# Rikorose/DeepFilterNet

Measured on AMD Instinct MI355X. Metric: 48 kHz audio frames/sec (hop=480), DeepFilterNet3 enhance(), higher is better.
Workload: dtype f32 (storage and accumulation; GRU projections / recurrences, the fused DF-encoder convolutions and the pointwise halves of the ERB separable convolutions as fp16-split MFMAs: x = hi + lo in f16, hi*hi + hi*lo + lo*hi on v_mfma_f32_16x16x32_f16, ~2^-21 relative; see exact_fp32_ms_per_step); 1 GPU; DeepFilterNet3 (recalled shipped shape, conv_ch=64) enhance(pad=True), batch=256 clips x 10 s @48 kHz per GPU, 1002 STFT frames per clip; batch_per_gpu=256, global_batch=256, parallelism=clips sharded over 1 GPU(s); no collective, inputs_resident_in_hbm=True

## Files before the change

deepfilternet_amd/csrc/dfx_nn_kernels.h:

```cpp
#pragma once

#include "dfx_common.h"

#include <type_traits>

#define DFX_ACT_NONE 0
#define DFX_ACT_RELU 1
#define DFX_ACT_TANH 2
#define DFX_ACT_SIGMOID 3

static __device__ __forceinline__ float dfx_sigmoid(float x) { return 1.f / (1.f + expf(-x)); }
static __device__ __forceinline__ float dfx_act(float v, int act) {
    if (act == DFX_ACT_RELU) return fmaxf(v, 0.f);
    if (act == DFX_ACT_TANH) return tanhf(v);
    if (act == DFX_ACT_SIGMOID) return dfx_sigmoid(v);
    return v;
}

template <int I, int N, typename F>
static __device__ __forceinline__ void dfx_static_for(F &&f) {
    if constexpr (I < N) {
        f(std::integral_constant<int, I>{});
        dfx_static_for<I + 1, N>(f);
    }
// ... 333 lines not shown
#pragma unroll
        for (int ks = 0; ks < CPL; ++ks) areg[nt][ks] = A.wt[(16 * (ks >> 2) + 4 * q + (ks & 3)) * C + 16 * nt + jl];
    float4 bias0[NT], biasr[NT];
#pragma unroll
    for (int nt = 0; nt < NT; ++nt) {
        bias0[nt] = reinterpret_cast<const float4 *>(A.bias0)[4 * nt + q];
        biasr[nt] = reinterpret_cast<const float4 *>(A.bias)[4 * nt + q];
    }
    __syncthreads();
    const int64_t Tn = A.t_end - A.t_begin;
    const int64_t total = A.B * Tn * A.Fout;
    const int64_t ntiles = (total + 15) / 16;
    for (int64_t tile = (int64_t)blockIdx.x * 4 + wave; tile < ntiles; tile += (int64_t)gridDim.x * 4) {
        const int64_t lpos = tile * 16 + jl;
        const bool valid = lpos < total;
        const int64_t rl = lpos / A.Fout;
        const int fo = (int)(lpos - rl * A.Fout);
        const int64_t b = rl / Tn, t = A.t_begin + (rl - b * Tn);
        const int64_t pos = (b * A.T + t) * A.Fout + fo;
        float u[CPL];
#pragma unroll
        for (int i = 0; i < CPL; ++i) u[i] = 0.f;
#pragma unroll
        for (int j = 0; j < 3; ++j) {
            const int fi = fo * A.stride + j - 1;
            const bool ok = valid && fi >= 0 && fi < A.Fin;
            float bv[5], c0v[CPL];
            dfx_c0_patch(A.feat, b, t, fi, ok, A.T, A.Fin, A.L, q, bv);
            dfx_c0_tile<C>(areg0, bias0, bv, ok, c0v);
#pragma unroll
            for (int nt = 0; nt < NT; ++nt) {
                const float4 w = dws[j * (C / 4) + 4 * nt + q];
                u[4 * nt + 0] += w.x * c0v[4 * nt + 0];
                u[4 * nt + 1] += w.y * c0v[4 * nt + 1];
                u[4 * nt + 2] += w.z * c0v[4 * nt + 2];
                u[4 * nt + 3] += w.w * c0v[4 * nt + 3];
            }
        }
        f32x4 acc[NT];
#pragma unroll
        for (int nt = 0; nt < NT; ++nt) acc[nt] = f32x4{0.f, 0.f, 0.f, 0.f};
#pragma unroll
        for (int ks = 0; ks < CPL; ++ks)
#pragma unroll
            for (int nt = 0; nt < NT; ++nt) acc[nt] = __builtin_amdgcn_mfma_f32_16x16x4f32(areg[nt][ks], u[ks], acc[nt], 0, 0, 0);
        if (valid) {
            float4 *op = reinterpret_cast<float4 *>(A.out + pos * C + 4 * q);
#pragma unroll
            for (int nt = 0; nt < NT; ++nt)
                op[4 * nt] = make_float4(fmaxf(acc[nt][0] + biasr[nt].x, 0.f), fmaxf(acc[nt][1] + biasr[nt].y, 0.f),
                                         fmaxf(acc[nt][2] + biasr[nt].z, 0.f), fmaxf(acc[nt][3] + biasr[nt].w, 0.f));
        }
    }
}

static __device__ __forceinline__ void dfx_c0_patch_load(const float *__restrict__ feat, int64_t b, int64_t t, int f, bool valid,
                                                         int64_t T, int Fin, int L, int q, float2 (&raw)[4], int64_t Ts = 0) {
    if (Ts <= 0) Ts = T;
#pragma unroll
    for (int i = 0; i < 4; ++i) {
        const int tap = 4 * q + i, kt = tap / 3, kf = tap - 3 * kt;
        const int64_t tau = t - 2 + kt, tin = tau + L;
        const int fin = f - 1 + kf;
        float2 v = make_float2(0.f, 0.f);
        if (valid && tap < 9 && tau >= 0 && tin < T && fin >= 0 && fin < Fin)
            v = *reinterpret_cast<const float2 *>(feat + ((b * Ts + tin) * Fin + fin) * 2);
        raw[i] = v;
    }
}

template <int C>
static __device__ __forceinline__ void dfx_c0_tile_h3(const dfx_h8 (&w0h)[C / 16], const dfx_h8 (&w0l)[C / 16],
                                                      const float4 (&bias0)[C / 16], float unscale0, const float2 (&raw)[4],
                                                      bool keep, float (&dst)[C / 4], float &amax) {
    constexpr int NT = C / 16;
    float x[8];
#pragma unroll
    for (int i = 0; i < 4; ++i) x[2 * i] = raw[i].x, x[2 * i + 1] = raw[i].y;
    dfx_h8 ph, pl;
    dfx_split8_g(x, ph, pl, amax);
    f32x4 acc[NT];
#pragma unroll
    for (int nt = 0; nt < NT; ++nt) acc[nt] = dfx_mfma_16x16x32_f16(w0l[nt], ph, f32x4{0.f, 0.f, 0.f, 0.f});
#pragma unroll
    for (int nt = 0; nt < NT; ++nt) acc[nt] = dfx_mfma_16x16x32_f16(w0h[nt], pl, acc[nt]);
#pragma unroll
    for (int nt = 0; nt < NT; ++nt) acc[nt] = dfx_mfma_16x16x32_f16(w0h[nt], ph, acc[nt]);
#pragma unroll
    for (int nt = 0; nt < NT; ++nt) {
        dst[4 * nt + 0] = keep ? fmaxf(acc[nt][0] * unscale0 + bias0[nt].x, 0.f) : 0.f;
        dst[4 * nt + 1] = keep ? fmaxf(acc[nt][1] * unscale0 + bias0[nt].y, 0.f) : 0.f;
        dst[4 * nt + 2] = keep ? fmaxf(acc[nt][2] * unscale0 + bias0[nt].z, 0.f) : 0.f;
        dst[4 * nt + 3] = keep ? fmaxf(acc[nt][3] * unscale0 + bias0[nt].w, 0.f) : 0.f;
    }
}

struct DfxC01hArgs {
    const float *feat;
    const dfx_h8 *w0f;
    const float *bias0;
    const float *dw;
    const dfx_h8 *wpf;
    const float *bias;
    float *out;
    int64_t B, T;
    int Fin, Fout, stride, L;
    float unscale0, unscale;
    int64_t t_begin;
    int64_t t_end;
    unsigned int *err;
    int64_t feat_T = 0;
};

template <int C>
#ifndef DFX_C01_MINB
#define DFX_C01_MINB 3
#endif
#ifndef DFX_C01_PIN
#define DFX_C01_PIN 0
#endif
#ifndef DFX_C01_EPI_BATCH
#define DFX_C01_EPI_BATCH 2
#endif
__global__ void __launch_bounds__(DFX_PW_THREADS, DFX_C01_MINB) dfx_k_df_conv01_h3(DfxC01hArgs A) {
    constexpr int CPL = C / 4, NT = C / 16, KC = C >= 32 ? C / 32 : 1, C4 = C / 4;
    static_assert(C % 32 == 0, "one k-chunk is 32 channels");
    __shared__ float4 dws[3 * C4];
    __shared__ float4 b0s[C4], b1s[C4];
    __shared__ dfx_h8 wps[NT * KC * 2 * 64];
    const int tid = threadIdx.x, lane = tid & 63, wave = tid >> 6, q = lane >> 4, jl = lane & 15;
    for (int i = tid; i < 3 * C4; i += DFX_PW_THREADS) dws[i] = reinterpret_cast<const float4 *>(A.dw)[i];
    for (int i = tid; i < C4; i += DFX_PW_THREADS) {
        b0s[i] = reinterpret_cast<const float4 *>(A.bias0)[i];
        b1s[i] = reinterpret_cast<const float4 *>(A.bias)[i];
    }
    for (int i = tid; i < NT * KC * 2 * 64; i += DFX_PW_THREADS) wps[i] = A.wpf[i];
    dfx_h8 w0h[NT], w0l[NT];
#pragma unroll
    for (int nt = 0; nt < NT; ++nt) {
        w0h[nt] = A.w0f[(nt * 2 + 0) * 64 + lane];
        w0l[nt] = A.w0f[(nt * 2 + 1) * 64 + lane];
    }
    __syncthreads();
    const unsigned Tn = (unsigned)(A.t_end - A.t_begin);
    const unsigned NF = (unsigned)A.B * Tn;
    const int TPF = (A.Fout + 15) >> 4;
    const unsigned nwaves = gridDim.x * 4;
    const int T32 = (int)A.T, Fin = A.Fin, Lk = A.L;
    int tdt[4], tdf[4];
    bool tok[4];
#pragma unroll
    for (int i = 0; i < 4; ++i) {
        const int tap = 4 * q + i, kt = tap / 3;
        tok[i] = tap < 9;
        tdt[i] = kt - 2 + Lk;
        tdf[i] = tap - 3 * kt - 1;
    }
    float2 raw[3][4];
    bool okj[3];
    const unsigned wid = (unsigned)blockIdx.x * 4 + (unsigned)dfx_wave_uniform(wave);
    const unsigned step_fr = nwaves / (unsigned)TPF;
    const int step_ft = (int)(nwaves - step_fr * (unsigned)TPF);
    unsigned nfr = wid / (unsigned)TPF;
    int nft = (int)(wid - nfr * (unsigned)TPF), nb = 0, nt_ = 0;
    bool nlive = nfr < NF;
    auto settle = [&]() {
        if (nlive) {
            nb = (int)(nfr / Tn);
            nt_ = (int)A.t_begin + (int)(nfr - (unsigned)nb * Tn);
        }
    };
    settle();
    auto issue = [&](int j) {
        const int fo = nft * 16 + jl;
        const int fi = fo * A.stride + j - 1;
        okj[j] = nlive && fo < A.Fout && fi >= 0 && fi < Fin;
        const float2 *clip = reinterpret_cast<const float2 *>(A.feat) + (int64_t)nb * (A.feat_T > 0 ? A.feat_T : (int64_t)T32) * Fin;
#pragma unroll
        for (int i = 0; i < 4; ++i) {
            const int tin = nt_ + tdt[i], fin = fi + tdf[i];
            float2 v = make_float2(0.f, 0.f);
            if (okj[j] && tok[i] && tin - Lk >= 0 && tin < T32 && fin >= 0 && fin < Fin) v = clip[tin * Fin + fin];
            raw[j][i] = v;
        }
    };
    float amax = 0.f;
#pragma unroll
    for (int j = 0; j < 3; ++j) issue(j);
    while (nlive) {
        const int fo_c = nft * 16 + jl;
        const bool valid = fo_c < A.Fout;
        const int64_t pos = ((int64_t)nb * T32 + nt_) * A.Fout + fo_c;
        nft += step_ft;
        nfr += step_fr;
        if (nft >= TPF) nft -= TPF, ++nfr;
        nlive = nfr < NF;
        settle();
        float u[CPL];
#pragma unroll
        for (int i = 0; i < CPL; ++i) u[i] = 0.f;
#pragma unroll
        for (int j = 0; j < 3; ++j) {
            float x[8];
#pragma unroll
            for (int i = 0; i < 4; ++i) x[2 * i] = raw[j][i].x, x[2 * i + 1] = raw[j][i].y;
            const bool keep = okj[j];
            dfx_h8 ph, pl;
            dfx_split8_g(x, ph, pl, amax);
            issue(j);
            f32x4 acc[NT];
#pragma unroll
            for (int nt = 0; nt < NT; ++nt) acc[nt] = dfx_mfma_16x16x32_f16(w0l[nt], ph, f32x4{0.f, 0.f, 0.f, 0.f});
#pragma unroll
            for (int nt = 0; nt < NT; ++nt) acc[nt] = dfx_mfma_16x16x32_f16(w0h[nt], pl, acc[nt]);
#pragma unroll
            for (int nt = 0; nt < NT; ++nt) acc[nt] = dfx_mfma_16x16x32_f16(w0h[nt], ph, acc[nt]);
#if DFX_C01_PIN
#pragma unroll
            for (int n0 = 0; n0 < NT; n0 += DFX_C01_EPI_BATCH) {
                float4 bz[DFX_C01_EPI_BATCH], w[DFX_C01_EPI_BATCH];
#pragma unroll
                for (int d = 0; d < DFX_C01_EPI_BATCH; ++d) {
                    bz[d] = b0s[4 * (n0 + d) + q], w[d] = dws[j * C4 + 4 * (n0 + d) + q];
                    DFX_OPAQUE(bz[d].x);
                    DFX_OPAQUE(bz[d].y);
                    DFX_OPAQUE(bz[d].z);
                    DFX_OPAQUE(bz[d].w);
                    DFX_OPAQUE(w[d].x);
                    DFX_OPAQUE(w[d].y);
                    DFX_OPAQUE(w[d].z);
                    DFX_OPAQUE(w[d].w);
                }
#pragma unroll
                for (int d = 0; d < DFX_C01_EPI_BATCH; ++d) {
                    const int nt = n0 + d;
                    u[4 * nt + 0] += w[d].x * (keep ? fmaxf(acc[nt][0] * A.unscale0 + bz[d].x, 0.f) : 0.f);
                    u[4 * nt + 1] += w[d].y * (keep ? fmaxf(acc[nt][1] * A.unscale0 + bz[d].y, 0.f) : 0.f);
                    u[4 * nt + 2] += w[d].z * (keep ? fmaxf(acc[nt][2] * A.unscale0 + bz[d].z, 0.f) : 0.f);
                    u[4 * nt + 3] += w[d].w * (keep ? fmaxf(acc[nt][3] * A.unscale0 + bz[d].w, 0.f) : 0.f);
                }
            }
#else
#pragma unroll
            for (int nt = 0; nt < NT; ++nt) {
                const float4 bz = b0s[4 * nt + q], w = dws[j * C4 + 4 * nt + q];
                u[4 * nt + 0] += w.x * (keep ? fmaxf(acc[nt][0] * A.unscale0 + bz.x, 0.f) : 0.f);
                u[4 * nt + 1] += w.y * (keep ? fmaxf(acc[nt][1] * A.unscale0 + bz.y, 0.f) : 0.f);
                u[4 * nt + 2] += w.z * (keep ? fmaxf(acc[nt][2] * A.unscale0 + bz.z, 0.f) : 0.f);
                u[4 * nt + 3] += w.w * (keep ? fmaxf(acc[nt][3] * A.unscale0 + bz.w, 0.f) : 0.f);
            }
#endif
        }
        dfx_h8 uh[KC], ul[KC];
#pragma unroll
        for (int kc = 0; kc < KC; ++kc) dfx_split8_g(u + 8 * kc, uh[kc], ul[kc], amax);
        float4 *op = reinterpret_cast<float4 *>(A.out + pos * C + 4 * q);
        int zoff = 0;
        DFX_OPAQUE(zoff);
        const dfx_h8 *wpl_ = wps + lane + zoff;
#pragma unroll
        for (int nt = 0; nt < NT; ++nt) {
            f32x4 aa = f32x4{0.f, 0.f, 0.f, 0.f}, ab = aa, ac = aa;
#pragma unroll
            for (int kc = 0; kc < KC; ++kc) {
                const dfx_h8 wh = wpl_[((nt * KC + kc) * 2 + 0) * 64], wl = wpl_[((nt * KC + kc) * 2 + 1) * 64];
                aa = dfx_mfma_16x16x32_f16(wl, uh[kc], aa);
                ab = dfx_mfma_16x16x32_f16(wh, ul[kc], ab);
                ac = dfx_mfma_16x16x32_f16(wh, uh[kc], ac);
            }
            if (valid) {
                const float4 bz = b1s[4 * nt + q];
                op[4 * nt] = make_float4(fmaxf(((aa[0] + ab[0]) + ac[0]) * A.unscale + bz.x, 0.f),
                                         fmaxf(((aa[1] + ab[1]) + ac[1]) * A.unscale + bz.y, 0.f),
                                         fmaxf(((aa[2] + ab[2]) + ac[2]) * A.unscale + bz.z, 0.f),
                                         fmaxf(((aa[3] + ab[3]) + ac[3]) * A.unscale + bz.w, 0.f));
            }
        }
    }
    if (amax >= DFX_H3_LIMIT && A.err) dfx_raise(A.err + 1);
}

struct DfxDfEncArgs {
    const float *feat;
    const dfx_h8 *w0f;
    const float *bias0;
    const float *dw;
    const dfx_h8 *wpf;
    const float *bias;
    const dfx_h8 *wfc;
    const dfx_h8 *win;
    const float *e3;
    float *emb_in;
    float *xa;
    int64_t B, T;
    int Fin, Fout, stride, L;
    int cpg;
    int nsplit = 1;
    float unscale0, unscale, unscale_fc, unscale_in;
    int64_t t_begin, t_end;
    unsigned int *err;
    int64_t feat_T = 0;
};

template <int C>
__global__ void __launch_bounds__(DFX_PW_THREADS, 3) dfx_k_df_enc_h3(DfxDfEncArgs A) {
    constexpr int CPL = C / 4, NT = C / 16, KC = C / 32, C4 = C / 4;
    static_assert(C % 32 == 0, "one k-chunk is 32 channels");
    __shared__ float4 dws[3 * C4];
    __shared__ float4 b0s[C4], b1s[C4];
    __shared__ dfx_h8 wps[NT * KC * 2 * 64];
    __shared__ dfx_h8 w0s[NT * 2 * 64];
    __shared__ __attribute__((aligned(16))) int tis[4 * DFX_PW_THREADS];
    __shared__ float4 uns[NT * DFX_PW_THREADS];
    const int tid = threadIdx.x, lane = tid & 63, wave = tid >> 6, q = lane >> 4, jl = lane & 15;
    for (int i = tid; i < 3 * C4; i += DFX_PW_THREADS) dws[i] = reinterpret_cast<const float4 *>(A.dw)[i];
    for (int i = tid; i < C4; i += DFX_PW_THREADS) {
        b0s[i] = reinterpret_cast<const float4 *>(A.bias0)[i];
        b1s[i] = reinterpret_cast<const float4 *>(A.bias)[i];
    }
    for (int i = tid; i < NT * KC * 2 * 64; i += DFX_PW_THREADS) wps[i] = A.wpf[i];
    for (int i = tid; i < NT * 2 * 64; i += DFX_PW_THREADS) w0s[i] = A.w0f[i];
    __syncthreads();
    const unsigned Tn = (unsigned)(A.t_end - A.t_begin), NFR = (unsigned)A.B * Tn, nsp = (unsigned)A.nsplit, ntiles = ((NFR + 15) >> 4) * nsp;
    const int bpp = A.Fout / A.nsplit;
    const unsigned nwaves = gridDim.x * 4;
    const int T32 = (int)A.T, Fin = A.Fin, Lk = A.L, Fout = A.Fout, emb = Fout * C / A.cpg / 2;
    const int64_t fT = A.feat_T > 0 ? A.feat_T : (int64_t)T32;
    {
        int ti[4];
#pragma unroll
        for (int i = 0; i < 4; ++i) {
            const int tap = 4 * q + i, kt = tap / 3;
            ti[i] = (kt - 2 + Lk + 64) | ((tap - 3 * kt) << 8) | ((tap < 9 ? 1 : 0) << 16);
        }
#pragma unroll
        for (int i = 0; i < 4; ++i) tis[4 * tid + i] = ti[i];
    }
    float amax = 0.f;
    for (unsigned tile = (unsigned)blockIdx.x * 4 + (unsigned)dfx_wave_uniform(wave); tile < ntiles; tile += nwaves) {
        const unsigned ftile = tile / nsp, part = tile - ftile * nsp;
        const int fo0 = (int)part * bpp, fo1 = fo0 + bpp;
        const unsigned rl = (ftile << 4) + (unsigned)jl, b = rl / Tn;
        const int t = (int)A.t_begin + (int)(rl - b * Tn);
        const bool live = rl < NFR;
        const float2 *feat2 = reinterpret_cast<const float2 *>(A.feat);
        const unsigned cbase = b * (unsigned)fT * (unsigned)Fin;
        const unsigned row = b * (unsigned)T32 + (unsigned)t;
        float2 raw[2][4];
        auto issue_to = [&](float2 (&dst)[4], int j, int fo) {
            const int fi = fo * A.stride + j - 1;
            const bool ok = live && fo < fo1 && fi >= 0 && fi < Fin;
            int zt = tid;
            DFX_OPAQUE(zt);
            const int tinfo[4] = {tis[4 * zt], tis[4 * zt + 1], tis[4 * zt + 2], tis[4 * zt + 3]};
#pragma unroll
            for (int i = 0; i < 4; ++i) {
                const int tin = t + (tinfo[i] & 0xff) - 64, fin = fi + ((tinfo[i] >> 8) & 0xff) - 1;
                float2 v = make_float2(0.f, 0.f);
                if (ok && (tinfo[i] >> 16) && tin - Lk >= 0 && tin < T32 && fin >= 0 && fin < Fin) v = feat2[cbase + (unsigned)(tin * Fin + fin)];
                dst[i] = v;
            }
        };
        auto c0_tile = [&](auto jc, auto addc, auto nextc, int fo, float2 (&rw)[4], float (&u)[CPL], bool refill) {
            constexpr int j = decltype(jc)::value;
            constexpr bool ADD = decltype(addc)::value, NEXT = decltype(nextc)::value;
            float x[8];
#pragma unroll
            for (int i = 0; i < 4; ++i) x[2 * i] = rw[i].x, x[2 * i + 1] = rw[i].y;
            const int fi = fo * A.stride + j - 1;
            const bool keep = live && fi >= 0 && fi < Fin;
            dfx_h8 ph, pl;
            dfx_split8_g(x, ph, pl, amax);
            if (refill) issue_to(rw, j, fo + 1);
            int z0 = 0;
            DFX_OPAQUE(z0);
            dfx_h8 w0h[NT], w0l[NT];
#pragma unroll
            for (int nt = 0; nt < NT; ++nt) {
                w0h[nt] = w0s[(nt * 2 + 0) * 64 + lane + z0];
                w0l[nt] = w0s[(nt * 2 + 1) * 64 + lane + z0];
            }
            f32x4 acc[NT];
#pragma unroll
            for (int nt = 0; nt < NT; ++nt) acc[nt] = dfx_mfma_16x16x32_f16(w0l[nt], ph, f32x4{0.f, 0.f, 0.f, 0.f});
#pragma unroll
            for (int nt = 0; nt < NT; ++nt) acc[nt] = dfx_mfma_16x16x32_f16(w0h[nt], pl, acc[nt]);
#pragma unroll
            for (int nt = 0; nt < NT; ++nt) acc[nt] = dfx_mfma_16x16x32_f16(w0h[nt], ph, acc[nt]);
#pragma unroll
            for (int nt = 0; nt < NT; ++nt) {
                const float4 bz = b0s[4 * nt + q];
                const float v0 = keep ? fmaxf(acc[nt][0] * A.unscale0 + bz.x, 0.f) : 0.f, v1 = keep ? fmaxf(acc[nt][1] * A.unscale0 + bz.y, 0.f) : 0.f;
                const float v2 = keep ? fmaxf(acc[nt][2] * A.unscale0 + bz.z, 0.f) : 0.f, v3 = keep ? fmaxf(acc[nt][3] * A.unscale0 + bz.w, 0.f) : 0.f;
                if constexpr (ADD) {
                    const float4 w = dws[j * C4 + 4 * nt + q];
                    u[4 * nt + 0] += w.x * v0;
                    u[4 * nt + 1] += w.y * v1;
                    u[4 * nt + 2] += w.z * v2;
                    u[4 * nt + 3] += w.w * v3;
                }
                if constexpr (NEXT) {
                    const float4 wn = dws[4 * nt + q];
                    uns[nt * DFX_PW_THREADS + tid] = make_float4(0.f + wn.x * v0, 0.f + wn.y * v1, 0.f + wn.z * v2, 0.f + wn.w * v3);
                }
            }
        };
        using I0 = std::integral_constant<int, 0>;
        using I1 = std::integral_constant<int, 1>;
        using I2 = std::integral_constant<int, 2>;
        f32x4 accg = f32x4{0.f, 0.f, 0.f, 0.f};
        float ev[8];
        int ci = fo0 * KC;
        {
            float none[CPL];
            issue_to(raw[0], 0, fo0);
            c0_tile(I0{}, std::false_type{}, std::true_type{}, fo0, raw[0], none, false);
            issue_to(raw[0], 1, fo0);
            issue_to(raw[1], 2, fo0);
        }
        for (int fo = fo0; fo < fo1; ++fo) {
            float u[CPL];
#pragma unroll
            for (int nt = 0; nt < NT; ++nt) {
                const float4 c = uns[nt * DFX_PW_THREADS + tid];
                u[4 * nt + 0] = c.x, u[4 * nt + 1] = c.y, u[4 * nt + 2] = c.z, u[4 * nt + 3] = c.w;
            }
            c0_tile(I1{}, std::true_type{}, std::false_type{}, fo, raw[0], u, true);
            c0_tile(I2{}, std::true_type{}, std::true_type{}, fo, raw[1], u, true);
            dfx_h8 uh[KC], ul[KC];
#pragma unroll
            for (int kc = 0; kc < KC; ++kc) dfx_split8_g(u + 8 * kc, uh[kc], ul[kc], amax);
            int zoff = 0;
            DFX_OPAQUE(zoff);
            const dfx_h8 *wpl_ = wps + lane + zoff;
#pragma unroll
            for (int kc = 0; kc < KC; ++kc, ++ci) {
                int lz = lane;
                DFX_OPAQUE(lz);
                const dfx_h8 *wfl_ = A.wfc + lz;
                const dfx_h8 fh = wfl_[((size_t)ci * 2 + 0) * 64], fl = wfl_[((size_t)ci * 2 + 1) * 64];
                float c1v[8];
#pragma unroll
                for (int h = 0; h < 2; ++h) {
                    const int nt = 2 * kc + h;
                    f32x4 aa = f32x4{0.f, 0.f, 0.f, 0.f}, ab = aa, ac = aa;
#pragma unroll
                    for (int k2 = 0; k2 < KC; ++k2) {
                        const dfx_h8 wh = wpl_[((nt * KC + k2) * 2 + 0) * 64], wl = wpl_[((nt * KC + k2) * 2 + 1) * 64];
                        aa = dfx_mfma_16x16x32_f16(wl, uh[k2], aa);
                        ab = dfx_mfma_16x16x32_f16(wh, ul[k2], ab);
                        ac = dfx_mfma_16x16x32_f16(wh, uh[k2], ac);
                    }
                    const float4 bz = b1s[4 * nt + q];
                    c1v[4 * h + 0] = fmaxf(((aa[0] + ab[0]) + ac[0]) * A.unscale + bz.x, 0.f);
                    c1v[4 * h + 1] = fmaxf(((aa[1] + ab[1]) + ac[1]) * A.unscale + bz.y, 0.f);
                    c1v[4 * h + 2] = fmaxf(((aa[2] + ab[2]) + ac[2]) * A.unscale + bz.z, 0.f);
                    c1v[4 * h + 3] = fmaxf(((aa[3] + ab[3]) + ac[3]) * A.unscale + bz.w, 0.f);
                }
                dfx_h8 ch, cl;
                dfx_split8_g(c1v, ch, cl, amax);
                accg = dfx_mfma_16x16x32_f16(fl, ch, accg);
                accg = dfx_mfma_16x16x32_f16(fh, cl, accg);
                accg = dfx_mfma_16x16x32_f16(fh, ch, accg);
                if ((ci + 1) % A.cpg == 0) {
                    const int g = ci / A.cpg;
                    float4 e = make_float4(0.f, 0.f, 0.f, 0.f);
                    if (live) e = *reinterpret_cast<const float4 *>(A.e3 + (row * (unsigned)emb + (unsigned)(16 * g + 4 * q)));
                    const float4 v = make_float4(fmaxf(accg[0] * A.unscale_fc, 0.f) + e.x, fmaxf(accg[1] * A.unscale_fc, 0.f) + e.y,
                                                 fmaxf(accg[2] * A.unscale_fc, 0.f) + e.z, fmaxf(accg[3] * A.unscale_fc, 0.f) + e.w);
                    if (A.emb_in && live) *reinterpret_cast<float4 *>(A.emb_in + (row * (unsigned)emb + (unsigned)(16 * g + 4 * q))) = v;
                    accg = f32x4{0.f, 0.f, 0.f, 0.f};
                    if (g & 1) {
                        ev[4] = v.x, ev[5] = v.y, ev[6] = v.z, ev[7] = v.w;
                        const int jg = g >> 1;
                        const dfx_h8 *wil_ = A.win + lane + zoff;
                        const dfx_h8 ih = wil_[((size_t)jg * 2 + 0) * 64], il = wil_[((size_t)jg * 2 + 1) * 64];
                        dfx_h8 eh, el;
                        dfx_split8_g(ev, eh, el, amax);
                        f32x4 o = dfx_mfma_16x16x32_f16(il, eh, f32x4{0.f, 0.f, 0.f, 0.f});
                        o = dfx_mfma_16x16x32_f16(ih, el, o);
                        o = dfx_mfma_16x16x32_f16(ih, eh, o);
                        if (live)
                            *reinterpret_cast<float4 *>(A.xa + (row * (unsigned)(emb / 2) + (unsigned)(16 * jg + 4 * q))) =
                                make_float4(fmaxf(o[0] * A.unscale_in, 0.f), fmaxf(o[1] * A.unscale_in, 0.f), fmaxf(o[2] * A.unscale_in, 0.f),
                                            fmaxf(o[3] * A.unscale_in, 0.f));
                    } else {
                        ev[0] = v.x, ev[1] = v.y, ev[2] = v.z, ev[3] = v.w;
                    }
                }
            }
        }
    }
    if (amax >= DFX_H3_LIMIT && A.err) dfx_raise(A.err + 1);
}

struct DfxCphArgs {
    const float *feat;
    const dfx_h8 *w0f;
    const float *bias0;
    const dfx_h8 *wf;
    const float *bias;
    float *out;
    int64_t B, T;
    int Fd, NO, nfb, nseg, tseg, L;
    float unscale0, unscale;
    int64_t t_begin, t_zero, t_end;
    unsigned int *err;
    int64_t feat_T = 0;
};

template <int C, int KT>
__global__ void __launch_bounds__(256, 1) dfx_k_df_convp_h3(DfxCphArgs A) {
    constexpr int CPL = C / 4, NT = C / 16, KC = C >= 32 ? C / 32 : 1;
    static_assert(C % 32 == 0, "one k-chunk is 32 channels");
    const int tid = threadIdx.x, lane = tid & 63, wave = tid >> 6, q = lane >> 4, jl = lane & 15;
    float4 bias0[NT];
#pragma unroll
    for (int nt = 0; nt < NT; ++nt) bias0[nt] = reinterpret_cast<const float4 *>(A.bias0)[4 * nt + q];
    dfx_h8 w0h[NT], w0l[NT], wh[KT][KC], wl[KT][KC];
#pragma unroll
    for (int nt = 0; nt < NT; ++nt) {
        w0h[nt] = A.w0f[(nt * 2 + 0) * 64 + lane];
        w0l[nt] = A.w0f[(nt * 2 + 1) * 64 + lane];
    }
#pragma unroll
    for (int k = 0; k < KT; ++k)
#pragma unroll
        for (int kc = 0; kc < KC; ++kc) {
            wh[k][kc] = A.wf[((k * KC + kc) * 2 + 0) * 64 + lane];
            wl[k][kc] = A.wf[((k * KC + kc) * 2 + 1) * 64 + lane];
            DFX_PIN_AGPR(wh[k][kc]);
            DFX_PIN_AGPR(wl[k][kc]);
        }
    float biasr[4];
#pragma unroll
    for (int r = 0; r < 4; ++r) biasr[r] = A.bias[4 * q + r];
    const int64_t nruns = A.B * A.nfb * A.nseg;
    float amax = 0.f;
    const int Fd = A.Fd, T32 = (int)A.T, Lk = A.L;
    const int fT = (int)(A.feat_T > 0 ? A.feat_T : A.T);
    int toff[4], tdt[4], tdf[4];
#pragma unroll
    for (int i = 0; i < 4; ++i) {
        const int tap = 4 * q + i, kt = tap / 3;
        tdt[i] = tap < 9 ? kt - 2 + Lk : (1 << 20);
        tdf[i] = tap - 3 * kt - 1;
        toff[i] = (kt - 2 + Lk) * Fd + tdf[i];
    }
    const float2 *feat2 = reinterpret_cast<const float2 *>(A.feat);
    for (int64_t run = (int64_t)blockIdx.x * 4 + dfx_wave_uniform(wave); run < nruns; run += (int64_t)gridDim.x * 4) {
        const int seg = (int)(run % A.nseg);
        const int64_t rest = run / A.nseg;
        const int fb = (int)(rest % A.nfb);
        const int64_t b = rest / A.nfb;
        const int f = fb * 16 + jl;
        const bool fvalid = f < Fd;
        const int64_t t0 = A.t_begin + (int64_t)seg * A.tseg;
        const int64_t t1 = (t0 + A.tseg < A.t_end) ? t0 + A.tseg : A.t_end;
        const unsigned cbase = (unsigned)b * (unsigned)fT * (unsigned)Fd;
        auto patch = [&](int t, bool ok, float2 (&rw)[4]) {
            const unsigned pbase = cbase + (unsigned)(t * Fd + f);
#pragma unroll
            for (int i = 0; i < 4; ++i) {
                const int tin = t + tdt[i], fin = f + tdf[i];
                const bool in = ok && tin - Lk >= 0 && tin < T32 && fin >= 0 && fin < Fd;
                const float2 v = feat2[in ? pbase + (unsigned)toff[i] : cbase];
                rw[i] = make_float2(in ? v.x : 0.f, in ? v.y : 0.f);
            }
        };
        dfx_h8 xh[KT][KC], xl[KT][KC];
        float2 raw[4];
        auto make_frame = [&](dfx_h8 (&dh)[KC], dfx_h8 (&dl)[KC], int64_t tau, const float2 (&rw)[4]) {
            float c0v[CPL];
            dfx_c0_tile_h3<C>(w0h, w0l, bias0, A.unscale0, rw, fvalid && tau >= A.t_zero, c0v, amax);
#pragma unroll
            for (int kc = 0; kc < KC; ++kc) dfx_split8_g(c0v + 8 * kc, dh[kc], dl[kc], amax);
        };
        dfx_static_for<1, KT>([&](auto sc) {
            constexpr int sl = decltype(sc)::value;
            const int64_t tau = t0 - KT + sl;
            patch((int)tau, fvalid && tau >= 0, raw);
            make_frame(xh[sl], xl[sl], tau, raw);
        });
        patch((int)t0, fvalid, raw);
        for (int64_t tb = t0; tb < t1; tb += KT) {
            dfx_static_for<0, KT>([&](auto pc) {
                constexpr int ph = decltype(pc)::value;
                const int64_t t = tb + ph;
                if (t < t1) {
                    float2 cur[4];
#pragma unroll
                    for (int i = 0; i < 4; ++i) cur[i] = raw[i];
                    patch((int)t + 1, fvalid && t + 1 < t1, raw);
                    make_frame(xh[ph], xl[ph], t, cur);
                    f32x4 aa = f32x4{0.f, 0.f, 0.f, 0.f}, ab = aa, ac = aa;
                    dfx_static_for<0, KT>([&](auto kcn) {
                        constexpr int k = decltype(kcn)::value;
                        constexpr int sl = (ph + 1 + k) % KT;
#pragma unroll
                        for (int kc = 0; kc < KC; ++kc) {
                            const dfx_h8 whk = wh[k][kc], wlk = wl[k][kc];
                            aa = dfx_mfma_16x16x32_f16(wlk, xh[sl][kc], aa);
                            ab = dfx_mfma_16x16x32_f16(whk, xl[sl][kc], ab);
                            ac = dfx_mfma_16x16x32_f16(whk, xh[sl][kc], ac);
                        }
                    });
                    f32x4 acc;
#pragma unroll
                    for (int r = 0; r < 4; ++r) acc[r] = (aa[r] + ab[r]) + ac[r];
                    if (fvalid) {
                        float *op = A.out + ((b * (A.NO / 2) * A.T + t) * A.Fd + f) * 2;
#pragma unroll
                        for (int h = 0; h < 2; ++h)
                            if (4 * q + 2 * h < A.NO)
                                *reinterpret_cast<float2 *>(op + (int64_t)(2 * q + h) * A.T * A.Fd * 2) =
                                    make_float2(fmaxf(acc[2 * h] * A.unscale + biasr[2 * h], 0.f),
                                                fmaxf(acc[2 * h + 1] * A.unscale + biasr[2 * h + 1], 0.f));
                    }
                }
            });
        }
    }
    if (amax >= DFX_H3_LIMIT && A.err) dfx_raise(A.err + 1);
}

template <int C, int KT, bool REBUILD>
__global__ void __launch_bounds__(256, REBUILD ? 1 : 2) dfx_k_df_convp_step(DfxCphArgs A, f32x4 *pend, int slot_new, const unsigned char *par = nullptr,
                                                             const int *cnt = nullptr) {
    constexpr int CPL = C / 4, NT = C / 16, KC = C / 32, NS = KT - 1;
    static_assert(C % 32 == 0 && KT >= 2, "one k-chunk is 32 channels; kt = 1 has no history");
    const int tid = threadIdx.x, lane = tid & 63, wave = tid >> 6, q = lane >> 4, jl = lane & 15;
    dfx_h8 w0h[NT], w0l[NT];
    float4 bias0[NT];
#pragma unroll
    for (int nt = 0; nt < NT; ++nt) {
        w0h[nt] = A.w0f[(nt * 2 + 0) * 64 + lane];
        w0l[nt] = A.w0f[(nt * 2 + 1) * 64 + lane];
        bias0[nt] = reinterpret_cast<const float4 *>(A.bias0)[4 * nt + q];
    }
    float biasr[4];
#pragma unroll
    for (int r = 0; r < 4; ++r) biasr[r] = A.bias[4 * q + r];
    const int64_t nruns = A.B * A.nfb;
    const int64_t t = A.T - 1;
    float amax = 0.f;
    for (int64_t run = (int64_t)blockIdx.x * 4 + wave; run < nruns; run += (int64_t)gridDim.x * 4) {
        const int fb = (int)(run % A.nfb);
        const int64_t b = run / A.nfb;
        const int f = fb * 16 + jl;
        const bool fvalid = f < A.Fd;
        const int half_in = par ? (int)(par[b] & 1) : 0, half_out = par ? half_in ^ 1 : 0, halves = par ? 2 : 1;
        const int slot0 = cnt ? cnt[b] % NS : slot_new;
        auto slot_ptr = [&](int j, int half) { return pend + ((((size_t)b * halves + half) * NS + (slot0 + j) % NS) * A.nfb + fb) * 64 + lane; };
        f32x4 sa[KT], sb[KT], sc[KT];
#pragma unroll
        for (int o = 0; o < KT; ++o) sa[o] = sb[o] = f32x4{0.f, 0.f, 0.f, 0.f}, sc[o] = f32x4{0.f, 0.f, 0.f, 0.f};
        if (!REBUILD) {
#pragma unroll
            for (int o = 0; o < NS; ++o) sc[o] = *slot_ptr(o, half_in);
        }
        dfx_static_for<(REBUILD ? 0 : KT - 1), KT>([&](auto dc) {
            constexpr int d = decltype(dc)::value;
            const int64_t tau = t - (KT - 1) + d;
            float2 raw[4];
            dfx_c0_patch_load(A.feat, b, tau, f, fvalid && tau >= 0, A.T, A.Fd, A.L, q, raw, A.feat_T);
            float c0v[CPL];
            dfx_c0_tile_h3<C>(w0h, w0l, bias0, A.unscale0, raw, fvalid && tau >= A.t_zero, c0v, amax);
            dfx_h8 xh[KC], xl[KC];
#pragma unroll
            for (int kc = 0; kc < KC; ++kc) dfx_split8_g(c0v + 8 * kc, xh[kc], xl[kc], amax);
            int zoff = 0;
            DFX_OPAQUE(zoff);
            const dfx_h8 *wfl = A.wf + lane + zoff;
#pragma unroll
            for (int kc = 0; kc < KC; ++kc) {
                dfx_h8 wl[KT], wh[KT];
                dfx_static_for<0, d + 1>([&](auto kcn) {
                    constexpr int k = decltype(kcn)::value;
                    wl[k] = wfl[((k * KC + kc) * 2 + 1) * 64], wh[k] = wfl[((k * KC + kc) * 2 + 0) * 64];
                });
                dfx_static_for<0, d + 1>([&](auto kcn) { constexpr int k = decltype(kcn)::value; sa[d - k] = dfx_mfma_16x16x32_f16(wl[k], xh[kc], sa[d - k]); });
                dfx_static_for<0, d + 1>([&](auto kcn) { constexpr int k = decltype(kcn)::value; sb[d - k] = dfx_mfma_16x16x32_f16(wh[k], xl[kc], sb[d - k]); });
                dfx_static_for<0, d + 1>([&](auto kcn) { constexpr int k = decltype(kcn)::value; sc[d - k] = dfx_mfma_16x16x32_f16(wh[k], xh[kc], sc[d - k]); });
            }
        });
        f32x4 sum[KT];
#pragma unroll
        for (int o = 0; o < KT; ++o)
#pragma unroll
            for (int r = 0; r < 4; ++r) sum[o][r] = (sa[o][r] + sb[o][r]) + sc[o][r];
#pragma unroll
        for (int o = 1; o < KT; ++o) *slot_ptr(o, half_out) = sum[o];
        if (fvalid) {
            float *op = A.out + ((b * (A.NO / 2) * A.T + t) * A.Fd + f) * 2;
#pragma unroll
            for (int h = 0; h < 2; ++h)
                if (4 * q + 2 * h < A.NO)
                    *reinterpret_cast<float2 *>(op + (int64_t)(2 * q + h) * A.T * A.Fd * 2) =
                        make_float2(fmaxf(sum[0][2 * h] * A.unscale + biasr[2 * h], 0.f), fmaxf(sum[0][2 * h + 1] * A.unscale + biasr[2 * h + 1], 0.f));
        }
    }
    if (amax >= DFX_H3_LIMIT && A.err) dfx_raise(A.err + 1);
}

#define DFX_CH_NF 2
template <int C, int MODE, typename Epi>
static __device__ __forceinline__ void dfx_chain_stage(const float *in, int Fin, int Fout, int stride, int npos,
                                                       const float4 *dws, const float (&areg)[C / 16][C / 4],
                                                       const float4 (&biasr)[C / 16], int lane, Epi &&epi) {
    constexpr int CPL = C / 4, NT = C / 16, V4 = CPL / 4, LD = C + 4;
    const int q = lane >> 4, jl = lane & 15;
    for (int p0 = 0; p0 < npos; p0 += 16) {
        const int p = p0 + jl;
        const bool valid = p < npos;
        const int fr = p / Fout, fo = p - fr * Fout;
        float u[CPL];
#pragma unroll
        for (int i = 0; i < CPL; ++i) u[i] = 0.f;
#pragma unroll
        for (int j = 0; j < 3; ++j) {
            int fi;
            bool ok;
            if (MODE == DFX_PW_MODE_DW3) {
                fi = fo * stride + j - 1;
                ok = fi >= 0 && fi < Fin;
            } else {
                const int num = fo + 1 - j;
                fi = num >> 1;
                ok = num >= 0 && (num & 1) == 0 && fi < Fin;
            }
            if (valid && ok) {
                const float4 *xp = reinterpret_cast<const float4 *>(in + (fr * Fin + fi) * LD + CPL * q);
#pragma unroll
                for (int v = 0; v < V4; ++v) {
                    const float4 xv = xp[v];
                    const float4 w = dws[j * (C / 4) + V4 * q + v];
                    u[4 * v + 0] += w.x * xv.x;
                    u[4 * v + 1] += w.y * xv.y;
                    u[4 * v + 2] += w.z * xv.z;
                    u[4 * v + 3] += w.w * xv.w;
                }
            }
        }
        f32x4 acc[NT];
#pragma unroll
        for (int nt = 0; nt < NT; ++nt) acc[nt] = f32x4{0.f, 0.f, 0.f, 0.f};
#pragma unroll
        for (int ks = 0; ks < CPL; ++ks)
#pragma unroll
            for (int nt = 0; nt < NT; ++nt) acc[nt] = __builtin_amdgcn_mfma_f32_16x16x4f32(areg[nt][ks], u[ks], acc[nt], 0, 0, 0);
#pragma unroll
        for (int nt = 0; nt < NT; ++nt)
            epi(p, valid, nt,
                make_float4(fmaxf(acc[nt][0] + biasr[nt].x, 0.f), fmaxf(acc[nt][1] + biasr[nt].y, 0.f),
                            fmaxf(acc[nt][2] + biasr[nt].z, 0.f), fmaxf(acc[nt][3] + biasr[nt].w, 0.f)));
    }
}

template <int C>
static __device__ __forceinline__ void dfx_chain_load_w(const float *wt, const float *bias, int lane, float (&areg)[C / 16][C / 4],
                                                        float4 (&biasr)[C / 16]) {
    constexpr int CPL = C / 4, NT = C / 16;
    const int q = lane >> 4, jl = lane & 15;
#pragma unroll
    for (int nt = 0; nt < NT; ++nt) {
#pragma unroll
        for (int ks = 0; ks < CPL; ++ks) areg[nt][ks] = wt[(CPL * q + ks) * C + 16 * nt + jl];
        biasr[nt] = reinterpret_cast<const float4 *>(bias)[4 * nt + q];
    }
}

template <int C>
static __device__ __forceinline__ void dfx_chain_load_w_h3(const dfx_h8 *frags, const float *bias, int lane, dfx_h8 (&ahi)[C / 16][C / 32],
                                                           dfx_h8 (&alo)[C / 16][C / 32], float4 (&biasr)[C / 16]) {
    constexpr int NT = C / 16, KC = C / 32;
    const int q = lane >> 4;
#pragma unroll
    for (int nt = 0; nt < NT; ++nt) {
#pragma unroll
        for (int kc = 0; kc < KC; ++kc) {
            ahi[nt][kc] = frags[((size_t)(nt * KC + kc) * 2 + 0) * 64 + lane];
            alo[nt][kc] = frags[((size_t)(nt * KC + kc) * 2 + 1) * 64 + lane];
        }
        biasr[nt] = reinterpret_cast<const float4 *>(bias)[4 * nt + q];
    }
}
template <int C, int MODE, typename Epi>
static __device__ __forceinline__ void dfx_chain_stage_h3(const float *in, int Fin, int Fout, int stride, int npos, const float4 *dws,
                                                          const dfx_h8 (&ahi)[C / 16][C / 32], const dfx_h8 (&alo)[C / 16][C / 32],
                                                          const float4 (&biasr)[C / 16], float unscale, float &amax, int lane, Epi &&epi) {
    constexpr int CPL = C / 4, NT = C / 16, KC = C / 32, V4 = CPL / 4, LD = C + 4;
    const int q = lane >> 4, jl = lane & 15;
    for (int p0 = 0; p0 < npos; p0 += 16) {
        const int p = p0 + jl;
        const bool valid = p < npos;
        const int fr = p / Fout, fo = p - fr * Fout;
        float u[CPL];
#pragma unroll
        for (int i = 0; i < CPL; ++i) u[i] = 0.f;
#pragma unroll
        for (int j = 0; j < 3; ++j) {
            int fi;
            bool ok;
            if (MODE == DFX_PW_MODE_DW3) {
                fi = fo * stride + j - 1;
                ok = fi >= 0 && fi < Fin;
            } else {
                const int num = fo + 1 - j;
                fi = num >> 1;
                ok = num >= 0 && (num & 1) == 0 && fi < Fin;
            }
            if (valid && ok) {
                const float4 *xp = reinterpret_cast<const float4 *>(in + (fr * Fin + fi) * LD + CPL * q);
#pragma unroll
                for (int v = 0; v < V4; ++v) {
                    const float4 xv = xp[v];
                    const float4 w = dws[j * (C / 4) + V4 * q + v];
                    u[4 * v + 0] += w.x * xv.x;
                    u[4 * v + 1] += w.y * xv.y;
                    u[4 * v + 2] += w.z * xv.z;
                    u[4 * v + 3] += w.w * xv.w;
                }
            }
        }
        dfx_h8 bhi[KC], blo[KC];
#pragma unroll
        for (int kc = 0; kc < KC; ++kc) dfx_split8_g(u + 8 * kc, bhi[kc], blo[kc], amax);
        f32x4 acc[NT];
#pragma unroll
        for (int nt = 0; nt < NT; ++nt) acc[nt] = f32x4{0.f, 0.f, 0.f, 0.f};
#pragma unroll
        for (int kc = 0; kc < KC; ++kc)
#pragma unroll
            for (int nt = 0; nt < NT; ++nt) {
                acc[nt] = dfx_mfma_16x16x32_f16(alo[nt][kc], bhi[kc], acc[nt]);
                acc[nt] = dfx_mfma_16x16x32_f16(ahi[nt][kc], blo[kc], acc[nt]);
                acc[nt] = dfx_mfma_16x16x32_f16(ahi[nt][kc], bhi[kc], acc[nt]);
            }
#pragma unroll
        for (int nt = 0; nt < NT; ++nt)
            epi(p, valid, nt,
                make_float4(fmaxf(acc[nt][0] * unscale + biasr[nt].x, 0.f), fmaxf(acc[nt][1] * unscale + biasr[nt].y, 0.f),
                            fmaxf(acc[nt][2] * unscale + biasr[nt].z, 0.f), fmaxf(acc[nt][3] * unscale + biasr[nt].w, 0.f)));
    }
}

#define DFX_PWF_MAXV 8
static __host__ __device__ __forceinline__ int dfx_pwf_group(int C, int Fin, int Fout) {
    int g = Fout < 16 && 16 % Fout == 0 ? 16 / Fout : 1;
    while (2 * g * Fin * (C / 4) <= 64 * 4 && 2 * g * Fout * (C / 4) <= 64 * DFX_PWF_MAXV) g *= 2;
    return g;
}
static __host__ __device__ __forceinline__ size_t dfx_pwf_wave_floats(int C, int Fin, int Fout) {
    return (size_t)dfx_pwf_group(C, Fin, Fout) * (size_t)(Fin + Fout) * (size_t)(C + 4);
}
static __host__ __device__ __forceinline__ size_t dfx_pwf_smem(int C, int Fin, int Fout) {
    return (size_t)(5 * C / 4) * 16 + 4 * dfx_pwf_wave_floats(C, Fin, Fout) * sizeof(float);
}
static __host__ __device__ __forceinline__ int dfx_pwf_nvi(int C, int Fin, int Fout) {
    return dfx_pwf_group(C, Fin, Fout) * Fin * (C / 4) <= 64 * 4 ? 4 : DFX_PWF_MAXV;
}
static __host__ __device__ __forceinline__ bool dfx_pwf_ok(int C, int Fin, int Fout) {
    const int G = dfx_pwf_group(C, Fin, Fout);
    return G * Fin * (C / 4) <= 64 * DFX_PWF_MAXV && G * Fout * (C / 4) <= 64 * DFX_PWF_MAXV && dfx_pwf_smem(C, Fin, Fout) <= 64 * 1024;
}

template <int C, int MODE, bool SKIP, int NVI , bool H3 = false>
__global__ void __launch_bounds__(DFX_PW_THREADS, (SKIP && NVI == DFX_PWF_MAXV) ? 1 : 2) dfx_k_pwconv_f(DfxPwArgs A) {
    constexpr int NT = C / 16, CPL = C / 4, LD = C + 4, C4 = C / 4, KC = H3 ? C / 32 : 1;
    DFX_DYN_SMEM(float4, dfx_pwf_smem4);
    float4 *dws = dfx_pwf_smem4, *sks = dfx_pwf_smem4 + 3 * C4;
    const int tid = threadIdx.x, lane = tid & 63, wave = tid >> 6, q = lane >> 4;
    const int G = dfx_pwf_group(C, A.Fin, A.Fout);
    const int nrow_in = G * A.Fin, npos = G * A.Fout;
    float *sin = reinterpret_cast<float *>(dfx_pwf_smem4 + 5 * C4) + (size_t)wave * dfx_pwf_wave_floats(C, A.Fin, A.Fout);
    float *sout = sin + (size_t)nrow_in * LD;
    for (int i = tid; i < 3 * C4; i += DFX_PW_THREADS) dws[i] = reinterpret_cast<const float4 *>(A.dw)[i];
    for (int i = tid; i < 2 * C4; i += DFX_PW_THREADS)
        sks[i] = SKIP ? (i < C4 ? reinterpret_cast<const float4 *>(A.sk_a)[i] : reinterpret_cast<const float4 *>(A.sk_b)[i - C4])
                      : make_float4(0.f, 0.f, 0.f, 0.f);
    float areg[H3 ? 1 : NT][H3 ? 1 : CPL];
    dfx_h8 ahi[NT][KC], alo[NT][KC];
    float4 biasr[NT];
    float amax = 0.f;
    if constexpr (H3) dfx_chain_load_w_h3<C>(A.wt_h3, A.bias, lane, ahi, alo, biasr);
    else dfx_chain_load_w<C>(A.wt, A.bias, lane, areg, biasr);
    __syncthreads();
    const int64_t nitems = (A.R + G - 1) / G;
    const int nin4 = nrow_in * C4, nout4 = npos * C4, fin4 = A.Fin * C4, fout4 = A.Fout * C4;
    const float4 *x4 = reinterpret_cast<const float4 *>(A.x);
    const float4 *s4 = reinterpret_cast<const float4 *>(A.skip);
    float4 *o4 = reinterpret_cast<float4 *>(A.out);
    float4 xr[NVI], sr[SKIP ? NVI : 1];
    const float inv_fin4 = 1.0f / (float)fin4, inv_fout = 1.0f / (float)A.Fout;
    auto issue = [&](int64_t item) {
        const int64_t base = item * G;
        const DfxRowBase rb = dfx_row_base(A.rm, base);
        int ln = lane;
        DFX_OPAQUE(ln);
        const float4 *xq = x4, *sq = s4;
#pragma unroll
        for (int i = 0; i < NVI; ++i) {
            const int idx = ln + 64 * i;
            xr[i] = make_float4(0.f, 0.f, 0.f, 0.f);
            if (SKIP) sr[i] = make_float4(0.f, 0.f, 0.f, 0.f);
            if (idx < nin4) {
                const int fr = dfx_div_small(idx, fin4, inv_fin4);
                const int64_t rl = base + fr;
                if (rl < A.R) {
                    const int64_t off = dfx_row_at(A.rm, base, rb, fr) * fin4 + (idx - fr * fin4);
                    xr[i] = xq[off];
                    if (SKIP) sr[i] = sq[off];
                }
            }
        }
    };
    int64_t item = (int64_t)blockIdx.x * 4 + wave;
    if (item < nitems) issue(item);
    static_assert(64 % C4 == 0, "channel quad of a lane must not depend on the load index");
    const float4 ska = sks[lane % C4], skb = sks[C4 + lane % C4];
    for (; item < nitems; item += (int64_t)gridDim.x * 4) {
#pragma unroll
        for (int i = 0; i < NVI; ++i) {
            const int idx = lane + 64 * i;
// ... 3024 lines not shown
```

deepfilternet_amd/csrc/env_hip/dfx_env.h:

```cpp
#pragma once

#include <hip/hip_runtime.h>

#include <cstdint>
#include <cstdio>
#include <cstdlib>
#include <cstring>
#include <utility>

typedef float f32x4 __attribute__((ext_vector_type(4)));
typedef float f32x2 __attribute__((ext_vector_type(2)));
typedef float f32x16 __attribute__((ext_vector_type(16)));

#define DFX_DYN_SMEM(T, name)                                                        \
    extern __shared__ __attribute__((aligned(16))) unsigned char dfx_dyn_smem_raw[]; \
    T *name = reinterpret_cast<T *>(dfx_dyn_smem_raw)

template <typename... KArgs, typename... Args>
static inline void dfx_launch(void (*kernel)(KArgs...), dim3 grid, dim3 block, size_t shmem, hipStream_t stream,
                              Args &&...args) {
    hipLaunchKernelGGL(kernel, grid, block, shmem, stream, static_cast<KArgs>(args)...);
}

static inline int dfx_env_num_cus() {
    static int n = -1;
    if (n < 0) {
        int dev = 0;
        hipDeviceProp_t prop;
        if (hipGetDevice(&dev) == hipSuccess && hipGetDeviceProperties(&prop, dev) == hipSuccess)
            n = prop.multiProcessorCount;
        else
            n = 256;
    }
    return n;
}
static inline int dfx_env_num_xcds() { return dfx_env_num_cus() / 32; }
static inline bool dfx_env_is_emulator() { return false; }
static __device__ __forceinline__ int dfx_wave_uniform(int v) { return __builtin_amdgcn_readfirstlane(v); }
#define DFX_NT_LOAD(p) __builtin_nontemporal_load(p)
#define DFX_NT_STORE(v, p) __builtin_nontemporal_store(v, p)
static __device__ __forceinline__ int dfx_xcc_id() { return (int)__builtin_amdgcn_s_getreg((3 << 11) | 20); }
static inline hipError_t dfx_env_set_max_dyn_smem(const void *func, size_t bytes) {
    return hipFuncSetAttribute(func, hipFuncAttributeMaxDynamicSharedMemorySize, (int)bytes);
}

static inline hipError_t dfx_env_err_words_alloc(unsigned int **host, unsigned int **dev, size_t bytes) {
    void *h = nullptr, *d = nullptr;
    hipError_t e = hipHostMalloc(&h, bytes, hipHostMallocMapped | hipHostMallocCoherent);
    if (e != hipSuccess) return e;
    memset(h, 0, bytes);
    e = hipHostGetDevicePointer(&d, h, 0);
    if (e != hipSuccess) {
        (void)hipHostFree(h);
        return e;
    }
    *host = static_cast<unsigned int *>(h), *dev = static_cast<unsigned int *>(d);
    return hipSuccess;
}
static inline void dfx_env_err_words_free(unsigned int *host) {
    if (host) (void)hipHostFree(host);
}
static __device__ __forceinline__ void dfx_raise(unsigned int *word) { __hip_atomic_store(word, 1u, __ATOMIC_RELAXED, __HIP_MEMORY_SCOPE_SYSTEM); }

typedef _Float16 dfx_h8 __attribute__((ext_vector_type(8)));
static __device__ __host__ __forceinline__ uint16_t dfx_f32_to_f16_bits(float x) {
    const _Float16 h = (_Float16)x;
    uint16_t b;
    __builtin_memcpy(&b, &h, 2);
    return b;
}
static __device__ __host__ __forceinline__ float dfx_f16_bits_to_f32(uint16_t b) {
    _Float16 h;
    __builtin_memcpy(&h, &b, 2);
    return (float)h;
}
typedef _Float16 dfx_h2v __attribute__((ext_vector_type(2)));
typedef float dfx_f2v __attribute__((ext_vector_type(2)));
static __device__ __forceinline__ void dfx_split8(const float *x, dfx_h8 &hi, dfx_h8 &lo) {
#pragma unroll
    for (int i = 0; i < 8; i += 2) {
        const dfx_f2v v = {x[i], x[i + 1]};
        const dfx_h2v h = __builtin_convertvector(v, dfx_h2v);
        const dfx_f2v r = v - __builtin_convertvector(h, dfx_f2v);
        const dfx_h2v l = __builtin_convertvector(r, dfx_h2v);
        hi[i] = h[0], hi[i + 1] = h[1];
        lo[i] = l[0], lo[i + 1] = l[1];
    }
}
#define DFX_H3_LIMIT 6.0e4f
static __device__ __forceinline__ void dfx_split8_g(const float *x, dfx_h8 &hi, dfx_h8 &lo, float &amax) {
#ifndef DFX_NO_H3_GUARD
    amax = fmaxf(amax, fmaxf(fmaxf(fmaxf(fabsf(x[0]), fabsf(x[1])), fmaxf(fabsf(x[2]), fabsf(x[3]))),
                             fmaxf(fmaxf(fabsf(x[4]), fabsf(x[5])), fmaxf(fabsf(x[6]), fabsf(x[7])))));
#endif
    dfx_split8(x, hi, lo);
}
static __device__ __forceinline__ f32x4 dfx_mfma_16x16x32_f16(dfx_h8 a, dfx_h8 b, f32x4 c) {
#ifdef DFX_MFMA_K16
    typedef _Float16 dfx_h4v __attribute__((ext_vector_type(4)));
    const dfx_h4v a0 = {a[0], a[1], a[2], a[3]}, a1 = {a[4], a[5], a[6], a[7]}, b0 = {b[0], b[1], b[2], b[3]}, b1 = {b[4], b[5], b[6], b[7]};
    c = __builtin_amdgcn_mfma_f32_16x16x16f16(a0, b0, c, 0, 0, 0);
    return __builtin_amdgcn_mfma_f32_16x16x16f16(a1, b1, c, 0, 0, 0);
#else
    return __builtin_amdgcn_mfma_f32_16x16x32_f16(a, b, c, 0, 0, 0);
#endif
}

static __device__ __forceinline__ float dfx_lane_gather4(float v, unsigned byte_addr) {
    return __builtin_bit_cast(float, __builtin_amdgcn_ds_bpermute((int)byte_addr, __builtin_bit_cast(int, v)));
}
#define DFX_MUL24(a, b) __mul24((a), (b))
#define DFX_OPAQUE(x) asm volatile("" : "+v"(x))
#define DFX_ASSUME(c) __builtin_assume(c)
#define DFX_PIN_AGPR(x) asm volatile("" : "+a"(x))
#define DFX_SCHED_BARRIER() __builtin_amdgcn_sched_barrier(0)
#define DFX_MFMA_GUARD()                         \
    do {                                         \
        __builtin_amdgcn_sched_barrier(0);       \
        asm volatile("s_nop 7");                 \
        __builtin_amdgcn_sched_barrier(0);       \
    } while (0)
#define DFX_VMEM_DRAIN() asm volatile("s_waitcnt vmcnt(0)" ::: "memory")
#define DFX_L1_INV() asm volatile("buffer_inv sc0" ::: "memory")
#define DFX_SCHED_GROUP(mask, n) __builtin_amdgcn_sched_group_barrier(mask, n, 0)
#ifdef DFX_WAVE_SYNC_WAIT
#define DFX_WAVE_SYNC()                                          \
    do {                                                         \
        __builtin_amdgcn_fence(__ATOMIC_RELEASE, "wavefront");   \
        asm volatile("s_waitcnt lgkmcnt(0)" ::: "memory");       \
        __builtin_amdgcn_wave_barrier();                         \
        __builtin_amdgcn_fence(__ATOMIC_ACQUIRE, "wavefront");   \
    } while (0)
#else
#define DFX_WAVE_SYNC()                                          \
    do {                                                         \
        __builtin_amdgcn_fence(__ATOMIC_RELEASE, "wavefront");   \
        __builtin_amdgcn_wave_barrier();                         \
        __builtin_amdgcn_fence(__ATOMIC_ACQUIRE, "wavefront");   \
    } while (0)
#endif

static __device__ __forceinline__ float dfx_fast_exp(float x) { return __expf(x); }
#ifndef DFX_RCP_RN
static __device__ __forceinline__ float dfx_fast_rcp(float x) { return __builtin_amdgcn_rcpf(x); }
#else
static __device__ __forceinline__ float dfx_fast_rcp(float x) { return __frcp_rn(x); }
#endif
```

Measured before the change: 23.04 million frames/s.

## Rework fp16 split codegen, skip pre-start frame compute, hoist DF-encoder store addressing

```diff
diff --git a/deepfilternet_amd/csrc/dfx_nn_kernels.h b/deepfilternet_amd/csrc/dfx_nn_kernels.h
--- a/deepfilternet_amd/csrc/dfx_nn_kernels.h
+++ b/deepfilternet_amd/csrc/dfx_nn_kernels.h
@@ -659,6 +659,9 @@
     int64_t feat_T = 0;
 };
 
+#ifndef DFX_SPLIT8_G_CVT
+#define dfx_split8_g_cvt dfx_split8_g
+#endif
 template <int C>
 __global__ void __launch_bounds__(DFX_PW_THREADS, 3) dfx_k_df_enc_h3(DfxDfEncArgs A) {
     constexpr int CPL = C / 4, NT = C / 16, KC = C / 32, C4 = C / 4;
@@ -727,7 +730,7 @@
             const int fi = fo * A.stride + j - 1;
             const bool keep = live && fi >= 0 && fi < Fin;
             dfx_h8 ph, pl;
-            dfx_split8_g(x, ph, pl, amax);
+            dfx_split8_g_cvt(x, ph, pl, amax);
             if (refill) issue_to(rw, j, fo + 1);
             int z0 = 0;
             DFX_OPAQUE(z0);
@@ -786,7 +789,7 @@
             c0_tile(I2{}, std::true_type{}, std::true_type{}, fo, raw[1], u, true);
             dfx_h8 uh[KC], ul[KC];
 #pragma unroll
-            for (int kc = 0; kc < KC; ++kc) dfx_split8_g(u + 8 * kc, uh[kc], ul[kc], amax);
+            for (int kc = 0; kc < KC; ++kc) dfx_split8_g_cvt(u + 8 * kc, uh[kc], ul[kc], amax);
             int zoff = 0;
             DFX_OPAQUE(zoff);
             const dfx_h8 *wpl_ = wps + lane + zoff;
@@ -815,7 +818,7 @@
                     c1v[4 * h + 3] = fmaxf(((aa[3] + ab[3]) + ac[3]) * A.unscale + bz.w, 0.f);
                 }
                 dfx_h8 ch, cl;
-                dfx_split8_g(c1v, ch, cl, amax);
+                dfx_split8_g_cvt(c1v, ch, cl, amax);
                 accg = dfx_mfma_16x16x32_f16(fl, ch, accg);
                 accg = dfx_mfma_16x16x32_f16(fh, cl, accg);
                 accg = dfx_mfma_16x16x32_f16(fh, ch, accg);
@@ -833,7 +836,7 @@
                         const dfx_h8 *wil_ = A.win + lane + zoff;
                         const dfx_h8 ih = wil_[((size_t)jg * 2 + 0) * 64], il = wil_[((size_t)jg * 2 + 1) * 64];
                         dfx_h8 eh, el;
-                        dfx_split8_g(ev, eh, el, amax);
+                        dfx_split8_g_cvt(ev, eh, el, amax);
                         f32x4 o = dfx_mfma_16x16x32_f16(il, eh, f32x4{0.f, 0.f, 0.f, 0.f});
                         o = dfx_mfma_16x16x32_f16(ih, el, o);
                         o = dfx_mfma_16x16x32_f16(ih, eh, o);
@@ -915,23 +918,40 @@
         const int64_t t0 = A.t_begin + (int64_t)seg * A.tseg;
         const int64_t t1 = (t0 + A.tseg < A.t_end) ? t0 + A.tseg : A.t_end;
         const unsigned cbase = (unsigned)b * (unsigned)fT * (unsigned)Fd;
+        bool fin_ok[4];
+#pragma unroll
+        for (int i = 0; i < 4; ++i) fin_ok[i] = f + tdf[i] >= 0 && f + tdf[i] < Fd;
+        float2 *const orow0 = reinterpret_cast<float2 *>(A.out) + ((b * (A.NO / 2) + 2 * q) * A.T + t0) * A.Fd + f;
+        float2 *const orow1 = orow0 + A.T * A.Fd;
+        const bool st0 = fvalid && 4 * q < A.NO, st1 = fvalid && 4 * q + 2 < A.NO;
+        const unsigned tspan = T32 > Lk ? (unsigned)(T32 - Lk) : 0u;
         auto patch = [&](int t, bool ok, float2 (&rw)[4]) {
             const unsigned pbase = cbase + (unsigned)(t * Fd + f);
 #pragma unroll
             for (int i = 0; i < 4; ++i) {
-                const int tin = t + tdt[i], fin = f + tdf[i];
-                const bool in = ok && tin - Lk >= 0 && tin < T32 && fin >= 0 && fin < Fd;
+                const bool in = ok && (unsigned)(t + tdt[i] - Lk) < tspan && fin_ok[i];
                 const float2 v = feat2[in ? pbase + (unsigned)toff[i] : cbase];
                 rw[i] = make_float2(in ? v.x : 0.f, in ? v.y : 0.f);
             }
         };
         dfx_h8 xh[KT][KC], xl[KT][KC];
         float2 raw[4];
+        float ramax = 0.f;
         auto make_frame = [&](dfx_h8 (&dh)[KC], dfx_h8 (&dl)[KC], int64_t tau, const float2 (&rw)[4]) {
-            float c0v[CPL];
-            dfx_c0_tile_h3<C>(w0h, w0l, bias0, A.unscale0, rw, fvalid && tau >= A.t_zero, c0v, amax);
-#pragma unroll
-            for (int kc = 0; kc < KC; ++kc) dfx_split8_g(c0v + 8 * kc, dh[kc], dl[kc], amax);
+            if (tau >= A.t_zero) {
+                float c0v[CPL];
+                dfx_c0_tile_h3<C>(w0h, w0l, bias0, A.unscale0, rw, true, c0v, ramax);
+#pragma unroll
+                for (int kc = 0; kc < KC; ++kc) dfx_split8_g(c0v + 8 * kc, dh[kc], dl[kc], ramax);
+            } else {
+                float x[8];
+#pragma unroll
+                for (int i = 0; i < 4; ++i) x[2 * i] = rw[i].x, x[2 * i + 1] = rw[i].y;
+                dfx_h8 ph, pl;
+                dfx_split8_g(x, ph, pl, ramax);
+#pragma unroll
+                for (int kc = 0; kc < KC; ++kc) dh[kc] = dfx_h8{}, dl[kc] = dfx_h8{};
+            }
         };
         dfx_static_for<1, KT>([&](auto sc) {
             constexpr int sl = decltype(sc)::value;
@@ -965,18 +985,13 @@
                     f32x4 acc;
 #pragma unroll
                     for (int r = 0; r < 4; ++r) acc[r] = (aa[r] + ab[r]) + ac[r];
-                    if (fvalid) {
-                        float *op = A.out + ((b * (A.NO / 2) * A.T + t) * A.Fd + f) * 2;
-#pragma unroll
-                        for (int h = 0; h < 2; ++h)
-                            if (4 * q + 2 * h < A.NO)
-                                *reinterpret_cast<float2 *>(op + (int64_t)(2 * q + h) * A.T * A.Fd * 2) =
-                                    make_float2(fmaxf(acc[2 * h] * A.unscale + biasr[2 * h], 0.f),
-                                                fmaxf(acc[2 * h + 1] * A.unscale + biasr[2 * h + 1], 0.f));
-                    }
+                    const int dt = (int)(t - t0) * Fd;
+                    if (st0) orow0[dt] = make_float2(fmaxf(acc[0] * A.unscale + biasr[0], 0.f), fmaxf(acc[1] * A.unscale + biasr[1], 0.f));
+                    if (st1) orow1[dt] = make_float2(fmaxf(acc[2] * A.unscale + biasr[2], 0.f), fmaxf(acc[3] * A.unscale + biasr[3], 0.f));
                 }
             });
         }
+        if (fvalid) amax = fmaxf(amax, ramax);
     }
     if (amax >= DFX_H3_LIMIT && A.err) dfx_raise(A.err + 1);
 }
diff --git a/deepfilternet_amd/csrc/env_hip/dfx_env.h b/deepfilternet_amd/csrc/env_hip/dfx_env.h
--- a/deepfilternet_amd/csrc/env_hip/dfx_env.h
+++ b/deepfilternet_amd/csrc/env_hip/dfx_env.h
@@ -77,6 +77,33 @@
 typedef _Float16 dfx_h2v __attribute__((ext_vector_type(2)));
 typedef float dfx_f2v __attribute__((ext_vector_type(2)));
 static __device__ __forceinline__ void dfx_split8(const float *x, dfx_h8 &hi, dfx_h8 &lo) {
+    float one;
+    asm("s_mov_b32 %0, 1.0" : "=s"(one));
+#pragma unroll
+    for (int i = 0; i < 8; i += 2) {
+        const dfx_f2v v = {x[i], x[i + 1]};
+        const dfx_h2v h = __builtin_convertvector(v, dfx_h2v);
+        _Float16 l0 = (_Float16)__builtin_fmaf(v[0], one, -(float)h[0]);
+        asm("" : "+v"(l0));
+        const _Float16 l1 = (_Float16)__builtin_fmaf(v[1], one, -(float)h[1]);
+        hi[i] = h[0], hi[i + 1] = h[1];
+        lo[i] = l0, lo[i + 1] = l1;
+    }
+}
+#define DFX_H3_LIMIT 6.0e4f
+static __device__ __forceinline__ void dfx_split8_g(const float *x, dfx_h8 &hi, dfx_h8 &lo, float &amax) {
+#ifndef DFX_NO_H3_GUARD
+    amax = fmaxf(amax, fmaxf(fmaxf(fmaxf(fabsf(x[0]), fabsf(x[1])), fmaxf(fabsf(x[2]), fabsf(x[3]))),
+                             fmaxf(fmaxf(fabsf(x[4]), fabsf(x[5])), fmaxf(fabsf(x[6]), fabsf(x[7])))));
+#endif
+    dfx_split8(x, hi, lo);
+}
+#define DFX_SPLIT8_G_CVT 1
+static __device__ __forceinline__ void dfx_split8_g_cvt(const float *x, dfx_h8 &hi, dfx_h8 &lo, float &amax) {
+#ifndef DFX_NO_H3_GUARD
+    amax = fmaxf(amax, fmaxf(fmaxf(fmaxf(fabsf(x[0]), fabsf(x[1])), fmaxf(fabsf(x[2]), fabsf(x[3]))),
+                             fmaxf(fmaxf(fabsf(x[4]), fabsf(x[5])), fmaxf(fabsf(x[6]), fabsf(x[7])))));
+#endif
 #pragma unroll
     for (int i = 0; i < 8; i += 2) {
         const dfx_f2v v = {x[i], x[i + 1]};
@@ -86,14 +113,6 @@
         hi[i] = h[0], hi[i + 1] = h[1];
         lo[i] = l[0], lo[i + 1] = l[1];
     }
-}
-#define DFX_H3_LIMIT 6.0e4f
-static __device__ __forceinline__ void dfx_split8_g(const float *x, dfx_h8 &hi, dfx_h8 &lo, float &amax) {
-#ifndef DFX_NO_H3_GUARD
-    amax = fmaxf(amax, fmaxf(fmaxf(fmaxf(fabsf(x[0]), fabsf(x[1])), fmaxf(fabsf(x[2]), fabsf(x[3]))),
-                             fmaxf(fmaxf(fabsf(x[4]), fabsf(x[5])), fmaxf(fabsf(x[6]), fabsf(x[7])))));
-#endif
-    dfx_split8(x, hi, lo);
 }
 static __device__ __forceinline__ f32x4 dfx_mfma_16x16x32_f16(dfx_h8 a, dfx_h8 b, f32x4 c) {
 #ifdef DFX_MFMA_K16
```

Result: no change. 23.00 million frames/s (median of 3 runs) (-0.2%).
